# kuleshov-group/PlantCaduceus

Measured on AMD Instinct MI355X. Metric: 512-bp sequences/sec (zero-shot logits), PlantCaduceus_l32, higher is better.
Workload: dtype bf16; 1 GPU; PlantCaduceus_l32 (d_model=1024, n_layer=32) bf16 zero-shot SNP scoring: masked-LM forward of 1024 synthetic 512-bp windows per GPU per step (both strands), logits at index 255 -> softmax(a,c,g,t); synthetic checkpoint seed 1234; batch_per_gpu=1024, seq_len=512, parallelism=dp1 (batch-sharded, all_gather of [B,4])

## Files before the change

include/pcad.h:

```cpp
#ifndef PCAD_H
#define PCAD_H

#include <stddef.h>
#include <stdint.h>

#ifdef __cplusplus
extern "C" {
#endif

#define PCAD_VERSION 100
#define PCAD_MAX_VOCAB 8
#define PCAD_MAX_POSITIONS 16

typedef void* pcad_stream;
typedef struct pcad_engine* pcad_handle;

enum pcad_status {
    PCAD_OK = 0,
    PCAD_ERR_INVALID = -1,
    PCAD_ERR_UNBOUND = -2,
    PCAD_ERR_WORKSPACE = -3,
    PCAD_ERR_MISSING = -4,
    PCAD_ERR_HIP = -5
};
// ... 26 lines not shown
const char* pcad_last_error(void);
const char* pcad_build_hash(void);

int    pcad_create(const pcad_config* cfg, pcad_handle* out);
void   pcad_destroy(pcad_handle h);

int    pcad_set_option(pcad_handle h, const char* key, int64_t value);

enum pcad_status_bits { PCAD_STATUS_BAD_TOKEN = 1, PCAD_STATUS_BAD_POSITION = 2 };
int    pcad_set_status_buffer(pcad_handle h, int32_t* status);

size_t pcad_weight_arena_bytes(pcad_handle h);

int    pcad_bind_weights(pcad_handle h, const pcad_tensor* tensors, int n,
                         void* arena, size_t arena_bytes, pcad_stream stream);

size_t pcad_workspace_bytes(pcad_handle h, int batch, int seqlen);

int    pcad_forward(pcad_handle h, const int32_t* ids, int B, int L,
                    const int32_t* positions, int P,
                    void* hidden_out, float* logits_out,
                    void* workspace, size_t workspace_bytes, pcad_stream stream);

int    pcad_forward_at(pcad_handle h, const int32_t* ids, int B, int L, const int32_t* pos_per_seq,
                       void* hidden_out, float* logits_out,
                       void* workspace, size_t workspace_bytes, pcad_stream stream);

int    pcad_forward_all_hidden(pcad_handle h, const int32_t* ids, int B, int L,
                               void* all_hidden, void* hidden_out, float* logits_out,
                               void* workspace, size_t workspace_bytes, pcad_stream stream);

enum pcad_pooling { PCAD_POOL_MEAN = 0, PCAD_POOL_MAX = 1, PCAD_POOL_FIRST = 2, PCAD_POOL_LAST = 3 };
#define PCAD_MAX_LABELS 256
int    pcad_forward_pooled(pcad_handle h, const int32_t* ids, int B, int L, int pooling, const float* score_w, int num_labels,
                           float* pooled_out, float* logits_out, void* workspace, size_t workspace_bytes, pcad_stream stream);

enum pcad_kernel_class {
    PCAD_K_NORM = 0, PCAD_K_GEMM_IN, PCAD_K_CONV, PCAD_K_GEMM_X, PCAD_K_SCAN, PCAD_K_GEMM_OUT, PCAD_K_HEAD,
    PCAD_K_GEMM_OUT_RES,
    PCAD_K_RSTD,
    PCAD_NUM_KERNEL_CLASSES
};
typedef struct pcad_kernel_stat {
    char    name[32];
    int64_t launches;
    double  total_ms;
} pcad_kernel_stat;
int pcad_profile_enable(pcad_handle h, int on);
int pcad_profile_read(pcad_handle h, pcad_kernel_stat* out, int max_out);


int pcad_add_rmsnorm(const void* x, const void* residual_in, const float* weight,
                     void* y, void* residual_out, int64_t rows, int D, float eps,
                     int dtype, int res_dtype, pcad_stream stream);

int pcad_causal_conv1d_silu(const void* x, int64_t ldx, const float* w_fwd, const float* b_fwd,
                            const float* w_rev, const float* b_rev, void* y_fwd, void* y_rev,
                            int S, int L, int E, int dtype, pcad_stream stream);

size_t pcad_conv_xproj_scratch_bytes(int E, int dtype);
int pcad_conv_xproj_bidir(const void* x, const float* w_fwd, const float* b_fwd, const float* w_rev, const float* b_rev,
                          const void* Wx_fwd, const void* Wx_rev, void* scratch,
                          void* xc_fwd, void* dtl_fwd, float* bc_fwd, void* xc_rev, void* dtl_rev, float* bc_rev,
                          int S, int L, int E, int Rp, int dtype, pcad_stream stream);

int pcad_selective_scan(const void* u, const void* delta, const void* z, int64_t ldz, const float* bc,
                        const float* A, const float* Dskip, const float* delta_bias,
                        void* y, int S, int L, int E, int reverse, int accumulate,
                        int dtype, pcad_stream stream);

int pcad_selective_scan_dtproj(const void* u, const void* dt_low, int64_t lddt, const void* Wdt, int Rp,
                               const void* z, int64_t ldz, const float* bc,
                               const float* A, const float* Dskip, const float* delta_bias,
                               void* y, int S, int L, int E, int reverse, int accumulate,
                               int dtype, pcad_stream stream);

int pcad_gemm_nt(const void* A, int64_t lda, const void* W, int64_t ldw, void* C, int64_t ldc,
                 int64_t M, int N, int K, int dtype, int out_dtype, pcad_stream stream);

size_t pcad_gemm_nt_split_scratch_bytes(int64_t M, int N, int K);
int pcad_gemm_nt_split(const float* A, int64_t lda, const float* W, int64_t ldw, float* C, int64_t ldc, int64_t M, int N, int K,
                       void* scratch, size_t scratch_bytes, pcad_stream stream);

int pcad_gemm_nt_residual(const void* A, int64_t lda, const void* W, int64_t ldw, void* C, float* res, float* ssq,
                          int64_t M, int N, int K, int dtype, pcad_stream stream);

int pcad_gather_rows(const void* src, void* out, int B, int L, int E, const int32_t* positions, int P, int dtype,
                     pcad_stream stream);

int pcad_final_head(const void* h, const void* res, const float* norm_weight, const float* emb_f32, const int32_t* complement,
                    void* hidden_out, float* logits_out, int B, int L, int D, float eps, const int32_t* positions, int P,
                    const int32_t* pos_per_seq, int h_compact, const int32_t* ids, int32_t* status, int dtype, int res_dtype,
                    int res_fragment_layout, pcad_stream stream);

size_t pcad_pooled_head_scratch_bytes(int B, int L, int D, int pooling);
int pcad_pooled_head(const void* h, const void* res, const float* norm_weight, const float* score_w, int num_labels,
                     float* pooled_out, float* logits_out, int B, int L, int D, float eps, int pooling, const int32_t* ids,
                     int32_t* status, int dtype, int res_dtype, int res_fragment_layout, void* scratch, size_t scratch_bytes,
                     pcad_stream stream);

#ifdef __cplusplus
}
#endif
#endif
```

plantcaduceus_amd/csrc/api.hip:

```cpp
#include <hip/hip_runtime.h>

#include <cstdarg>
#include <cstdio>
#include <cstdlib>
#include <cstring>
#include <map>
#include <string>
#include <vector>

#include "../../include/pcad.h"
#include "build_hash.h"
#include "kernels.hpp"

using namespace pcad;

namespace {

thread_local char g_err[512] = "";

int fail(int code, const char* fmt, ...) {
    va_list ap;
    va_start(ap, fmt);
    vsnprintf(g_err, sizeof(g_err), fmt, ap);
    va_end(ap);
// ... 801 lines not shown
        return fail(PCAD_ERR_INVALID, "pcad_conv_xproj_bidir: null argument");
    if (dtype != PCAD_F32 && dtype != PCAD_BF16) return fail(PCAD_ERR_INVALID, "pcad_conv_xproj_bidir: bad dtype");
    if (Rp != 64 && Rp != 96) return fail(PCAD_ERR_INVALID, "pcad_conv_xproj_bidir: Rp must be 64 (dt_rank <= 64) or 96 (dt_rank 65..96)");
    const int64_t esz = dtype == PCAD_BF16 ? 2 : 4;
    if (S < 0 || L < 0 || E <= 0 || (E * esz) % 128)
        return fail(PCAD_ERR_INVALID, "pcad_conv_xproj_bidir: E * elem must be a multiple of 128 bytes");
    if (((int64_t)S * L + 16) * E * esz >= ((int64_t)1 << 32))
        return fail(PCAD_ERR_INVALID, "pcad_conv_xproj_bidir: (S*L + 16) * E * elem must be < 2^32 (32-bit in-tensor offsets)");
    if (S == 0 || L == 0) return PCAD_OK;
    hipStream_t s = (hipStream_t)stream;
    HIP_TRY(launch_pack_convw(w_fwd, b_fwd, w_rev, b_rev, (float*)scratch, E, dtype, s));
    HIP_TRY(launch_convx(x, (const float*)scratch, Wx_fwd, xc_fwd, dtl_fwd, bc_fwd, Wx_rev, xc_rev, dtl_rev, bc_rev, S, L, E,
                         dtype, s, Rp));
    return PCAD_OK;
}

static int scan_args_ok(const void* u, const float* bc, const float* A, const float* Dskip, const float* delta_bias,
                        void* y, int S, int L, int E) {
    if (!u || !bc || !A || !Dskip || !delta_bias || !y) return fail(PCAD_ERR_INVALID, "pcad_selective_scan: null argument");
    if (S < 0 || L < 0 || E <= 0 || E % 64) return fail(PCAD_ERR_INVALID, "pcad_selective_scan: E must be a multiple of 64");
    if (((uintptr_t)bc) % 16) return fail(PCAD_ERR_INVALID, "pcad_selective_scan: bc must be 16-byte aligned");
    return PCAD_OK;
}

int pcad_selective_scan(const void* u, const void* delta, const void* z, int64_t ldz, const float* bc, const float* A,
                        const float* Dskip, const float* delta_bias, void* y, int S, int L, int E, int reverse,
                        int accumulate, int dtype, pcad_stream stream) {
    if (!delta) return fail(PCAD_ERR_INVALID, "pcad_selective_scan: null delta");
    if (int rc = scan_args_ok(u, bc, A, Dskip, delta_bias, y, S, L, E)) return rc;
    if (S == 0 || L == 0) return PCAD_OK;
    HIP_TRY(launch_scan(u, z, ldz, delta, nullptr, 0, nullptr, 0, bc, A, 1.4426950408889634f, Dskip, delta_bias, y, S, L,
                        E, reverse != 0, accumulate, dtype, (hipStream_t)stream));
    return PCAD_OK;
}

int pcad_selective_scan_dtproj(const void* u, const void* dt_low, int64_t lddt, const void* Wdt, int Rp, const void* z,
                               int64_t ldz, const float* bc, const float* A, const float* Dskip,
                               const float* delta_bias, void* y, int S, int L, int E, int reverse, int accumulate,
                               int dtype, pcad_stream stream) {
    if (!dt_low || !Wdt) return fail(PCAD_ERR_INVALID, "pcad_selective_scan_dtproj: null dt_low / Wdt");
    if (Rp <= 0 || Rp % 32 || lddt < Rp || ((uintptr_t)dt_low) % 16 || ((uintptr_t)Wdt) % 16 ||
        (lddt * (dtype == PCAD_BF16 ? 2 : 4)) % 16)
        return fail(PCAD_ERR_INVALID, "pcad_selective_scan_dtproj: Rp must be a multiple of 32 (zero padded), rows 16-byte aligned");
    if (int rc = scan_args_ok(u, bc, A, Dskip, delta_bias, y, S, L, E)) return rc;
    if (S == 0 || L == 0) return PCAD_OK;
    HIP_TRY(launch_scan(u, z, ldz, nullptr, dt_low, lddt, Wdt, Rp, bc, A, 1.4426950408889634f, Dskip, delta_bias, y, S, L,
                        E, reverse != 0, accumulate, dtype, (hipStream_t)stream));
    return PCAD_OK;
}

int pcad_gemm_nt(const void* A, int64_t lda, const void* W, int64_t ldw, void* C, int64_t ldc, int64_t M, int N, int K,
                 int dtype, int out_dtype, pcad_stream stream) {
    if (!A || !W || !C) return fail(PCAD_ERR_INVALID, "pcad_gemm_nt: null argument");
    hipError_t err = launch_gemm_nt(A, lda, W, ldw, C, ldc, M, N, K, dtype, out_dtype, false, (hipStream_t)stream);
    if (err == hipErrorInvalidValue)
        return fail(PCAD_ERR_INVALID, "pcad_gemm_nt: K*elem must be a multiple of 128 bytes; A/W 16-byte aligned rows");
    if (err != hipSuccess) return fail(PCAD_ERR_HIP, "pcad_gemm_nt: %s", hipGetErrorString(err));
    return PCAD_OK;
}

size_t pcad_gemm_nt_split_scratch_bytes(int64_t M, int N, int K) {
    if (M <= 0 || N <= 0 || K <= 0) return 0;
    return align_up((size_t)M * 2 * K * 2) + align_up((size_t)N * 2 * K * 2);
}

int pcad_gemm_nt_split(const float* A, int64_t lda, const float* W, int64_t ldw, float* C, int64_t ldc, int64_t M, int N, int K,
                       void* scratch, size_t scratch_bytes, pcad_stream stream) {
    if (!A || !W || !C || !scratch) return fail(PCAD_ERR_INVALID, "pcad_gemm_nt_split: null argument");
    if (M < 0 || N <= 0 || K <= 0 || K % 64 || lda < K || ldw < K || ldc < N)
        return fail(PCAD_ERR_INVALID, "pcad_gemm_nt_split: K must be a multiple of 64; lda, ldw >= K; ldc >= N");
    if (((uintptr_t)scratch) % 256 || scratch_bytes < pcad_gemm_nt_split_scratch_bytes(M, N, K))
        return fail(PCAD_ERR_WORKSPACE, "pcad_gemm_nt_split: scratch must be 256-byte aligned and pcad_gemm_nt_split_scratch_bytes large");
    if (M == 0) return PCAD_OK;
    hipStream_t s = (hipStream_t)stream;
    void* As = scratch;
    void* Ws = (char*)scratch + align_up((size_t)M * 2 * K * 2);
    HIP_TRY(launch_split_rows(A, lda, As, M, K, false, false, s));
    HIP_TRY(launch_pack_split_w(W, PCAD_F32, ldw, Ws, N, K, s));
    hipError_t err = launch_gemm_nt(As, 2 * (int64_t)K, Ws, 2 * (int64_t)K, C, ldc, M, N, 3 * K, BF16, F32, false, s, false, K / 64);
    if (err != hipSuccess) return fail(PCAD_ERR_HIP, "pcad_gemm_nt_split: %s", hipGetErrorString(err));
    return PCAD_OK;
}

int pcad_gemm_nt_residual(const void* A, int64_t lda, const void* W, int64_t ldw, void* C, float* res, float* ssq, int64_t M, int N,
                          int K, int dtype, pcad_stream stream) {
    if (!A || !W || !res || !ssq || !C) return fail(PCAD_ERR_INVALID, "pcad_gemm_nt_residual: null argument");
    if (dtype != PCAD_F32 && dtype != PCAD_BF16) return fail(PCAD_ERR_INVALID, "pcad_gemm_nt_residual: bad dtype");
    if (M < 0 || N <= 0 || K <= 0 || M % 256 || N % 256 || M * (int64_t)N * 4 >= ((int64_t)1 << 32))
        return fail(PCAD_ERR_INVALID, "pcad_gemm_nt_residual: M and N must be multiples of 256 and M * N * 4 < 2^32");
    hipError_t err = launch_gemm_nt_res(A, lda, W, ldw, C, res, ssq, M, N, K, dtype, (hipStream_t)stream, false);
    if (err == hipErrorInvalidValue)
        return fail(PCAD_ERR_INVALID, "pcad_gemm_nt_residual: K*elem must be a multiple of 128 bytes; 16-byte aligned rows; tensors < 4 GiB");
    if (err != hipSuccess) return fail(PCAD_ERR_HIP, "pcad_gemm_nt_residual: %s", hipGetErrorString(err));
    return PCAD_OK;
}

static int positions_arg(const char* who, const int32_t* positions, int P, int L, Positions* pos) {
    if (P < 0 || P > PCAD_MAX_POSITIONS || (P > 0 && !positions)) return fail(PCAD_ERR_INVALID, "%s: bad positions (P=%d)", who, P);
    pos->n = P;
    for (int i = 0; i < 16; ++i) pos->p[i] = 0;
    for (int i = 0; i < P; ++i) {
        if (positions[i] < 0 || positions[i] >= L) return fail(PCAD_ERR_INVALID, "%s: position %d out of range [0,%d)", who, positions[i], L);
        pos->p[i] = positions[i];
    }
    return PCAD_OK;
}

int pcad_gather_rows(const void* src, void* out, int B, int L, int E, const int32_t* positions, int P, int dtype, pcad_stream stream) {
    if (!src || !out) return fail(PCAD_ERR_INVALID, "pcad_gather_rows: null argument");
    if (dtype != PCAD_F32 && dtype != PCAD_BF16) return fail(PCAD_ERR_INVALID, "pcad_gather_rows: bad dtype");
    if (B < 0 || L <= 0 || E <= 0 || (E * (dtype == PCAD_BF16 ? 2 : 4)) % 16 || P < 1)
        return fail(PCAD_ERR_INVALID, "pcad_gather_rows: bad shape (E * elem must be a multiple of 16 bytes, P >= 1)");
    Positions pos;
    if (int rc = positions_arg("pcad_gather_rows", positions, P, L, &pos)) return rc;
    if (B == 0) return PCAD_OK;
    HIP_TRY(launch_gather_rows(src, out, B, L, E, pos, dtype, false, (hipStream_t)stream));
    return PCAD_OK;
}

int pcad_final_head(const void* h, const void* res, const float* norm_weight, const float* emb_f32, const int32_t* complement,
                    void* hidden_out, float* logits_out, int B, int L, int D, float eps, const int32_t* positions, int P,
                    const int32_t* pos_per_seq, int h_compact, const int32_t* ids, int32_t* status, int dtype, int res_dtype,
                    int res_fragment_layout, pcad_stream stream) {
    if (!h || !res || !norm_weight || !emb_f32 || !complement) return fail(PCAD_ERR_INVALID, "pcad_final_head: null argument");
    if (res_fragment_layout && (res_dtype != PCAD_F32 || D % 256 || ((int64_t)2 * B * L) % 256))
        return fail(PCAD_ERR_INVALID, "pcad_final_head: the fragment layout needs an fp32 residual, D %% 256 == 0 and 2 B L %% 256 == 0");
    if ((dtype != PCAD_F32 && dtype != PCAD_BF16) || (res_dtype != PCAD_F32 && res_dtype != PCAD_BF16) || (dtype == PCAD_F32 && res_dtype != PCAD_F32))
        return fail(PCAD_ERR_INVALID, "pcad_final_head: bad dtype / res_dtype");
    if (B < 0 || L <= 0 || D <= 0 || D % 8 || D > 2048) return fail(PCAD_ERR_INVALID, "pcad_final_head: bad B / L / D");
    if (pos_per_seq && (positions || P)) return fail(PCAD_ERR_INVALID, "pcad_final_head: positions and pos_per_seq are exclusive");
    if (h_compact && (pos_per_seq || P == 0)) return fail(PCAD_ERR_INVALID, "pcad_final_head: h_compact needs a shared list of positions");
    Positions pos;
    if (int rc = positions_arg("pcad_final_head", positions, P, L, &pos)) return rc;
    if (B == 0) return PCAD_OK;
    HIP_TRY(launch_final_head(h, res, norm_weight, nullptr, emb_f32, complement, hidden_out, logits_out, B, L, D, eps, pos, pos_per_seq,
                              dtype, res_dtype, (hipStream_t)stream, h_compact != 0, ids, status, res_fragment_layout ? D : 0));
    return PCAD_OK;
}

size_t pcad_pooled_head_scratch_bytes(int B, int L, int D, int pooling) {
    if (B <= 0 || L <= 0 || D <= 0 || pooling < PCAD_POOL_MEAN || pooling > PCAD_POOL_LAST) return 0;
    return align_up(pool_partial_bytes(B, L, D, pooling));
}

int pcad_pooled_head(const void* h, const void* res, const float* norm_weight, const float* score_w, int num_labels,
                     float* pooled_out, float* logits_out, int B, int L, int D, float eps, int pooling, const int32_t* ids,
                     int32_t* status, int dtype, int res_dtype, int res_fragment_layout, void* scratch, size_t scratch_bytes,
                     pcad_stream stream) {
    if (!h || !res || !norm_weight || !scratch) return fail(PCAD_ERR_INVALID, "pcad_pooled_head: null argument");
    if (!pooled_out && !logits_out) return fail(PCAD_ERR_INVALID, "pcad_pooled_head: no output requested");
    if (logits_out && (!score_w || num_labels < 1 || num_labels > PCAD_MAX_LABELS))
        return fail(PCAD_ERR_INVALID, "pcad_pooled_head: logits need score_w and 1 <= num_labels <= %d", PCAD_MAX_LABELS);
    if (pooling < PCAD_POOL_MEAN || pooling > PCAD_POOL_LAST) return fail(PCAD_ERR_INVALID, "pcad_pooled_head: bad pooling %d", pooling);
    if (res_fragment_layout && (res_dtype != PCAD_F32 || D % 256 || ((int64_t)2 * B * L) % 256))
        return fail(PCAD_ERR_INVALID, "pcad_pooled_head: the fragment layout needs an fp32 residual, D %% 256 == 0 and 2 B L %% 256 == 0");
    if ((dtype != PCAD_F32 && dtype != PCAD_BF16) || (res_dtype != PCAD_F32 && res_dtype != PCAD_BF16) || (dtype == PCAD_F32 && res_dtype != PCAD_F32))
        return fail(PCAD_ERR_INVALID, "pcad_pooled_head: bad dtype / res_dtype");
    if (B < 0 || L <= 0 || D <= 0 || D % 8 || D > 2048) return fail(PCAD_ERR_INVALID, "pcad_pooled_head: bad B / L / D");
    if (B == 0) return PCAD_OK;
    if (((uintptr_t)scratch) % 256 || scratch_bytes < pcad_pooled_head_scratch_bytes(B, L, D, pooling))
        return fail(PCAD_ERR_WORKSPACE, "pcad_pooled_head: scratch must be 256-byte aligned and pcad_pooled_head_scratch_bytes large");
    HIP_TRY(launch_pooled_head(h, res, norm_weight, score_w, num_labels, pooled_out, logits_out, B, L, D, eps, pooling, ids, status,
                               dtype, res_dtype, res_fragment_layout ? D : 0, scratch, (hipStream_t)stream));
    return PCAD_OK;
}

// ... 2 lines not shown
```

plantcaduceus_amd/csrc/gemm.hip:

```cpp
#include <cstdlib>
#include <type_traits>

#include "common.hpp"
#include "kernels.hpp"

namespace pcad {

typedef __bf16 bf16x8_t __attribute__((ext_vector_type(8)));

constexpr int BM = 256, BN = 128, ROWB = 128;
constexpr int A_BYTES = BM * ROWB, W_BYTES = BN * ROWB;
constexpr int STAGE_BYTES = A_BYTES + W_BYTES;
constexpr int NSTAGE = 3;
constexpr int GEMM_LDS = NSTAGE * STAGE_BYTES;
constexpr int GEMM_THREADS = 512;
#ifndef PCAD_WALK_CONST
#define PCAD_WALK_CONST 8
#endif
constexpr int walk = PCAD_WALK_CONST;

__device__ __forceinline__ int ksplit_a(int kt, int nk) { return kt >= 2 * nk ? kt - 2 * nk : kt; }
__device__ __forceinline__ int ksplit_w(int kt, int nk) { return kt >= nk ? kt - nk : kt; }
__device__ __forceinline__ int key_a(int r) { return (r >> 1) & 7; }
__device__ __forceinline__ int key_w(int r) { return (((r >> 4) & 3) << 1) | ((r >> 1) & 1); }
// ... 801 lines not shown
                        *reinterpret_cast<u32x4*>(db + 64) = H;
                        __builtin_amdgcn_sched_barrier(0);
                        continue;
                    }
                }
                store8<OutT>(dst, lo);
                store8<OutT>(dst + 8, hi);
                __builtin_amdgcn_sched_barrier(0);
            }
        }
        if constexpr (EPI == EPI_RES) {
            const int np = N >> 7;
#pragma unroll
            for (int i = 0; i < 8; ++i) {
                float v = ss[i];
                v += __shfl_xor(v, 16, 64);
                v += __shfl_xor(v, 32, 64);
                if (lg == 0) epi.ssq[(mrow + i * 16) * np + (n0 >> 7) + wn] = v;
            }
        }
    };

    int tile = blockIdx.x;
    int64_t m0; int n0;
    tile_coords(tile, m0, n0);
    set_pa(m0);
    set_pw(n0);
    load_rscale(m0);
    a_issue(0); a_advance();
    w_issue(0); w_advance();
    a_issue(1); a_advance();
    w_issue(1); w_advance();
    asm volatile("s_waitcnt vmcnt(16)" ::: "memory");
    __builtin_amdgcn_s_barrier();
    asm volatile("" ::: "memory");
    u32x4 fa0[8], fw0[8], fa1[8], fw1[8];
    load_frags(0, 0, 0, fa0, fw0);
    int sa = 0, sw = 0, kt = 0;
    auto mainloop = [&](auto slot) __attribute__((always_inline)) {
    while (true) {
        const int sa_n = sa == 2 ? 0 : sa + 1;
        const int sa_f = sa == 0 ? 2 : sa - 1;
        if constexpr (EPI == EPI_RES) {
            if (kt == 0) {
                const float* tb = res_tile_base(m0, n0);
#pragma unroll
                for (int i = 0; i < 8; ++i) { load_res_group(tb, i, 0); load_res_group(tb, i, 1); }
                kstep(fa0, fw0, fa1, fw1, sa, sw, 1, true, sa_f, std::integral_constant<int, 2>{}, slot);
            } else {
                kstep(fa0, fw0, fa1, fw1, sa, sw, 1, true, sa_f, std::integral_constant<int, 0>{}, slot);
            }
        } else {
            if (kt == 0) kstep(fa0, fw0, fa1, fw1, sa, sw, 1, true, sa_f, std::integral_constant<int, 1>{}, slot);
            else kstep(fa0, fw0, fa1, fw1, sa, sw, 1, true, sa_f, std::integral_constant<int, 0>{}, slot);
        }
        a_advance();
        asm volatile("s_waitcnt vmcnt(8) lgkmcnt(0)" ::: "memory");
        __builtin_amdgcn_s_barrier();
        asm volatile("" ::: "memory");
        kstep(fa1, fw1, fa0, fw0, sa_n, sw ^ 1, 0, false, sw, std::integral_constant<int, 0>{}, slot);
        w_advance();
        sa = sa_n;
        sw ^= 1;
        if (kt + 1 < nkt) {
            ++kt;
        } else {
            epilogue(m0, n0);
            tile += gstride;
            if (tile >= nblk) break;
            tile_coords(tile, m0, n0);
            load_rscale(m0);
            kt = 0;
        }
    }
    };
#ifdef PCAD_GEMM_STAGGER
    if (wave == 0) mainloop(std::integral_constant<int, 0>{});
    else if (wave == 1) mainloop(std::integral_constant<int, 1>{});
    else if (wave == 2) mainloop(std::integral_constant<int, 2>{});
    else mainloop(std::integral_constant<int, 3>{});
#else
    mainloop(std::integral_constant<int, kDmaSlot>{});
#endif
    asm volatile("s_waitcnt vmcnt(0)" ::: "memory");
}

static int persistent_grid(int nblk) {
    const int cap = device_cu_count() / 8 * 8;
    return nblk < cap ? nblk : cap;
}

template <typename T, typename OutT, bool ROUND>
static hipError_t launch_gemm_t(const void* A, int64_t lda, const void* W, int64_t ldw, void* C, int64_t ldc,
                                int64_t M, int N, int K, hipStream_t s, bool a_blocked, int ksplit = 0) {
    const int tiles_m = (int)((M + BM - 1) / BM), tiles_n = (N + BN - 1) / BN;
    const bool vec = ((ldc * (int64_t)sizeof(OutT)) % 16 == 0) && (((uintptr_t)C) % 16 == 0);
    dim3 grid((unsigned)persistent_grid(tiles_m * tiles_n)), block(GEMM_THREADS);
    if (vec) {
        auto kfn = gemm_nt_kernel<T, OutT, ROUND, true, false>;
        if (hipError_t ae = ensure_dynamic_lds((const void*)kfn, GEMM_LDS)) return ae;
        hipLaunchKernelGGL(kfn, grid, block, GEMM_LDS, s, (const T*)A, lda, (const T*)W, ldw, (OutT*)C, ldc, M, N, K,
                           tiles_m, tiles_n, (float*)nullptr, (int64_t)0, 0, (int)a_blocked, ksplit);
    } else {
        auto kfn = gemm_nt_kernel<T, OutT, ROUND, false, false>;
        if (hipError_t ae = ensure_dynamic_lds((const void*)kfn, GEMM_LDS)) return ae;
        hipLaunchKernelGGL(kfn, grid, block, GEMM_LDS, s, (const T*)A, lda, (const T*)W, ldw, (OutT*)C, ldc, M, N, K,
                           tiles_m, tiles_n, (float*)nullptr, (int64_t)0, 0, (int)a_blocked, ksplit);
    }
    return hipGetLastError();
}

template <typename T>
static hipError_t launch_gemm_split_t(const void* A, int64_t lda, const void* W, int64_t ldw, void* C, int64_t ldc,
                                      float* C2, int64_t ldc2, int nsplit, int64_t M, int N, int K, hipStream_t s,
                                      bool a_blocked) {
    const int tiles_m = (int)((M + BM - 1) / BM), tiles_n = (N + BN - 1) / BN;
    dim3 grid((unsigned)persistent_grid(tiles_m * tiles_n)), block(GEMM_THREADS);
    auto kfn = gemm_nt_kernel<T, T, false, true, true>;
    if (hipError_t ae = ensure_dynamic_lds((const void*)kfn, GEMM_LDS)) return ae;
    hipLaunchKernelGGL(kfn, grid, block, GEMM_LDS, s, (const T*)A, lda, (const T*)W, ldw, (T*)C, ldc, M, N, K, tiles_m,
                       tiles_n, C2, ldc2, nsplit, (int)a_blocked, 0);
    return hipGetLastError();
}

hipError_t launch_gemm_nt_split(const void* A, int64_t lda, const void* W, int64_t ldw, void* C, int64_t ldc, float* C2,
                                int64_t ldc2, int nsplit, int64_t M, int N, int K, int dt, hipStream_t s, bool a_blocked) {
    if (M <= 0 || N <= 0) return hipSuccess;
    const int esz = dt == BF16 ? 2 : 4;
    if (K <= 0 || (K * esz) % ROWB || nsplit % 16 || (N - nsplit) % 16) return hipErrorInvalidValue;
    if ((lda * esz) % 16 || (ldw * esz) % 16 || ((uintptr_t)A) % 16 || ((uintptr_t)W) % 16) return hipErrorInvalidValue;
    if ((ldc * esz) % 16 || ((uintptr_t)C) % 16 || (ldc2 * 4) % 16 || ((uintptr_t)C2) % 16) return hipErrorInvalidValue;
    if (a_blocked && (lda * esz) % 128) return hipErrorInvalidValue;
    if (dt == BF16) return launch_gemm_split_t<bf16_t>(A, lda, W, ldw, C, ldc, C2, ldc2, nsplit, M, N, K, s, a_blocked);
    return launch_gemm_split_t<float>(A, lda, W, ldw, C, ldc, C2, ldc2, nsplit, M, N, K, s, a_blocked);
}

template <typename T>
static bool quad_ok(int64_t lda, int64_t ldw, int64_t M, int N, bool two, int nsplit) {
    const int64_t esz_ = (int64_t)sizeof(T);
    return M % BM2 == 0 && N % BN2 == 0 && (!two || nsplit % 64 == 0) && M * lda * esz_ < ((int64_t)1 << 32) - 65536 &&
           (int64_t)N * ldw * esz_ < ((int64_t)1 << 32) - 65536;
}

template <typename T, typename OutT = T>
static hipError_t launch_gemm256_t(const void* A, int64_t lda, const void* W, int64_t ldw, void* C, int64_t ldc, int64_t M,
                                   int N, int K, hipStream_t s, bool a_blocked, void* C2 = nullptr, int nsplit = 0,
                                   bool out_blocked = false, int epi_kind = EPI_NONE, GemmEpi epi = GemmEpi{nullptr, nullptr, nullptr},
                                   int ksplit = 0) {
    const int tiles_m = (int)((M + BM2 - 1) / BM2), tiles_n = (N + BN2 - 1) / BN2;
    dim3 grid((unsigned)persistent_grid(tiles_m * tiles_n)), block(GEMM_THREADS);
    static const bool quad = dev_env("PCAD_GEMM_NOQUAD") == nullptr;
    static const bool epi_swap = dev_env("PCAD_GEMM_EPI_PLAIN") == nullptr;
    const bool qok = quad_ok<T>(lda, ldw, M, N, C2 != nullptr, nsplit);
    if (epi_kind != EPI_NONE && !qok) return hipErrorInvalidValue;
#define PCAD_LAUNCH_Q(EPIK)                                                                                                     \
    do {                                                                                                                        \
        auto kq = gemm256q_kernel<T, OutT, EPIK>;                                                                               \
        if (hipError_t ae = ensure_dynamic_lds((const void*)kq, GEMM3_LDS)) return ae;                                          \
        hipLaunchKernelGGL(kq, grid, dim3(GEMMQ_THREADS), GEMM3_LDS, s, (const T*)A, lda, (const T*)W, ldw, (OutT*)C, ldc, M, N, K, \
                           tiles_m, tiles_n, (int)a_blocked, (OutT*)C2, nsplit, (int)out_blocked, (int)epi_swap, epi, ksplit); \
                                                                                             \
        return hipGetLastError();                                                                                               \
    } while (0)
    if constexpr (std::is_same<T, OutT>::value) {
        if (epi_kind == EPI_SCALE) PCAD_LAUNCH_Q(EPI_SCALE);
        if (epi_kind == EPI_RES) PCAD_LAUNCH_Q(EPI_RES);
    } else if (epi_kind != EPI_NONE) {
        return hipErrorInvalidValue;
    }
    if (quad && qok) PCAD_LAUNCH_Q(EPI_NONE);
#undef PCAD_LAUNCH_Q
    auto kr = gemm256r_kernel<T, OutT>;
    if (hipError_t ae = ensure_dynamic_lds((const void*)kr, GEMM3_LDS)) return ae;
    hipLaunchKernelGGL(kr, grid, block, GEMM3_LDS, s, (const T*)A, lda, (const T*)W, ldw, (OutT*)C, ldc, M, N, K, tiles_m,
                       tiles_n, (int)a_blocked, (OutT*)C2, nsplit, (int)out_blocked, ksplit);
    return hipGetLastError();
}

hipError_t launch_gemm_nt_two(const void* A, int64_t lda, const void* W, int64_t ldw, void* C1, void* C2, int nsplit,
                              bool out_blocked, int64_t M, int N, int K, int dt, hipStream_t s, const float* rscale, int out_dt, int ksplit) {
    if (M <= 0 || N <= 0) return hipSuccess;
    const int esz = dt == BF16 ? 2 : 4;
    if (out_dt < 0) out_dt = dt;
    const int osz = out_dt == BF16 ? 2 : 4;
    if (K <= 0 || (K * esz) % ROWB || nsplit % 16 || N % 16 || nsplit <= 0 || nsplit >= N) return hipErrorInvalidValue;
    if ((lda * esz) % 16 || (ldw * esz) % 16 || ((uintptr_t)A) % 16 || ((uintptr_t)W) % 16) return hipErrorInvalidValue;
    if (((uintptr_t)C1) % 16 || ((uintptr_t)C2) % 16) return hipErrorInvalidValue;
    if (out_blocked && ((nsplit * osz) % 128 || ((N - nsplit) * osz) % 128)) return hipErrorInvalidValue;
    const int ek = rscale ? EPI_SCALE : EPI_NONE;
    const GemmEpi epi{rscale, nullptr, nullptr};
    if (out_dt != dt) {
        if (dt != BF16 || out_dt != F32 || rscale) return hipErrorInvalidValue;
        if (ksplit && (ksplit < 0 || K != 3 * ksplit * (ROWB / 2))) return hipErrorInvalidValue;
        return launch_gemm256_t<bf16_t, float>(A, lda, W, ldw, C1, nsplit, M, N, K, s, false, C2, nsplit, out_blocked, EPI_NONE, epi, ksplit);
    }
    if (ksplit) return hipErrorInvalidValue;
    if (dt == BF16) return launch_gemm256_t<bf16_t>(A, lda, W, ldw, C1, nsplit, M, N, K, s, false, C2, nsplit, out_blocked, ek, epi);
    return launch_gemm256_t<float>(A, lda, W, ldw, C1, nsplit, M, N, K, s, false, C2, nsplit, out_blocked, ek, epi);
}

bool gemm_fold_shapes_ok(int64_t M, int D, int E, int dt) {
    const int64_t esz = dt == BF16 ? 2 : 4;
    const int Dp = fold_padded_width(D);
    const bool in_ok = dt == BF16 ? quad_ok<bf16_t>(Dp, D, M, 2 * E, true, E) : quad_ok<float>(Dp, D, M, 2 * E, true, E);
    const bool out_ok = dt == BF16 ? quad_ok<bf16_t>(E, E, M, Dp, false, 0) : quad_ok<float>(E, E, M, Dp, false, 0);
    return in_ok && out_ok && (D * esz) % ROWB == 0 && (E * esz) % ROWB == 0 && M * (int64_t)Dp * 4 < ((int64_t)1 << 32);
}

hipError_t launch_gemm_nt_res(const void* A, int64_t lda, const void* W, int64_t ldw, void* C, float* res, float* ssq, int64_t M,
                              int N, int K, int dt, hipStream_t s, bool a_blocked) {
    if (M <= 0 || N <= 0) return hipSuccess;
    const int esz = dt == BF16 ? 2 : 4;
    if (K <= 0 || (K * esz) % ROWB || !res || !ssq || !C) return hipErrorInvalidValue;
    if ((lda * esz) % 16 || (ldw * esz) % 16 || ((uintptr_t)A) % 16 || ((uintptr_t)W) % 16 || ((uintptr_t)res) % 16) return hipErrorInvalidValue;
    if (a_blocked && (lda * esz) % 128) return hipErrorInvalidValue;
    const GemmEpi epi{nullptr, res, ssq};
    if (dt == BF16) return launch_gemm256_t<bf16_t>(A, lda, W, ldw, C, N, M, N, K, s, a_blocked, nullptr, 0, false, EPI_RES, epi);
    return launch_gemm256_t<float>(A, lda, W, ldw, C, N, M, N, K, s, a_blocked, nullptr, 0, false, EPI_RES, epi);
}

hipError_t launch_gemm_nt(const void* A, int64_t lda, const void* W, int64_t ldw, void* C, int64_t ldc, int64_t M,
                          int N, int K, int dt, int out_dt, bool round_bf16, hipStream_t s, bool a_blocked, int ksplit) {
    if (M <= 0 || N <= 0) return hipSuccess;
    const int esz = dt == BF16 ? 2 : 4;
    if (K <= 0 || (K * esz) % ROWB) return hipErrorInvalidValue;
    if (ksplit && (ksplit < 0 || dt != BF16 || out_dt != F32 || round_bf16 || K != 3 * ksplit * (ROWB / 2))) return hipErrorInvalidValue;
    if ((lda * esz) % 16 || (ldw * esz) % 16 || ((uintptr_t)A) % 16 || ((uintptr_t)W) % 16)
        return hipErrorInvalidValue;
    if (a_blocked && (lda * esz) % 128) return hipErrorInvalidValue;
    static const bool no256 = dev_env("PCAD_GEMM_NO256") != nullptr;
    const int osz = out_dt == BF16 ? 2 : 4;
    const bool big = !no256 && M >= 2048 && N >= 512 && N % 16 == 0 && (out_dt == dt || (dt == BF16 && out_dt == F32 && !round_bf16)) &&
                     (ldc * osz) % 16 == 0 && ((uintptr_t)C) % 16 == 0;
    if (big) {
        if (dt == BF16 && out_dt == F32)
            return launch_gemm256_t<bf16_t, float>(A, lda, W, ldw, C, ldc, M, N, K, s, a_blocked, nullptr, 0, false, EPI_NONE, GemmEpi{nullptr, nullptr, nullptr}, ksplit);
        if (dt == BF16) return launch_gemm256_t<bf16_t>(A, lda, W, ldw, C, ldc, M, N, K, s, a_blocked);
        return launch_gemm256_t<float>(A, lda, W, ldw, C, ldc, M, N, K, s, a_blocked);
    }
    if (dt == BF16 && out_dt == BF16)
        return launch_gemm_t<bf16_t, bf16_t, false>(A, lda, W, ldw, C, ldc, M, N, K, s, a_blocked);
    if (dt == BF16 && out_dt == F32)
        return round_bf16 ? launch_gemm_t<bf16_t, float, true>(A, lda, W, ldw, C, ldc, M, N, K, s, a_blocked)
                          : launch_gemm_t<bf16_t, float, false>(A, lda, W, ldw, C, ldc, M, N, K, s, a_blocked, ksplit);
    if (dt == F32 && out_dt == F32)
        return launch_gemm_t<float, float, false>(A, lda, W, ldw, C, ldc, M, N, K, s, a_blocked);
    return hipErrorInvalidValue;
}

}
```

plantcaduceus_amd/engine.py:

```python
from __future__ import annotations

import ctypes as C
import os
import subprocess
from typing import Dict, Optional, Sequence

import torch

_HERE = os.path.dirname(os.path.abspath(__file__))
LIB_PATH = os.environ.get("PCAD_LIB") or os.path.join(_HERE, "libpcad.so")
CSRC = os.path.join(_HERE, "csrc")

PCAD_F32, PCAD_BF16 = 0, 1
_DT = {torch.float32: PCAD_F32, torch.bfloat16: PCAD_BF16}


class PcadConfig(C.Structure):
    _fields_ = [
        ("d_model", C.c_int32), ("n_layer", C.c_int32), ("d_state", C.c_int32), ("d_conv", C.c_int32),
        ("expand", C.c_int32), ("dt_rank", C.c_int32), ("vocab", C.c_int32), ("eps", C.c_float),
        ("dtype", C.c_int32), ("residual_in_fp32", C.c_int32), ("complement", C.c_int32 * 8),
    ]


class PcadKernelStat(C.Structure):
    _fields_ = [("name", C.c_char * 32), ("launches", C.c_int64), ("total_ms", C.c_double)]


class PcadTensor(C.Structure):
    _fields_ = [("name", C.c_char_p), ("data", C.c_void_p), ("dtype", C.c_int32), ("ndim", C.c_int32),
                ("shape", C.c_int64 * 4)]


SIGNATURES = {
    "pcad_version": (C.c_int, []),
    "pcad_last_error": (C.c_char_p, []),
    "pcad_build_hash": (C.c_char_p, []),
    "pcad_set_status_buffer": (C.c_int, [C.c_void_p, C.c_void_p]),
    "pcad_create": (C.c_int, [C.POINTER(PcadConfig), C.POINTER(C.c_void_p)]),
    "pcad_destroy": (None, [C.c_void_p]),
    "pcad_set_option": (C.c_int, [C.c_void_p, C.c_char_p, C.c_int64]),
    "pcad_weight_arena_bytes": (C.c_size_t, [C.c_void_p]),
    "pcad_bind_weights": (C.c_int, [C.c_void_p, C.POINTER(PcadTensor), C.c_int, C.c_void_p, C.c_size_t, C.c_void_p]),
    "pcad_workspace_bytes": (C.c_size_t, [C.c_void_p, C.c_int, C.c_int]),
    "pcad_forward": (C.c_int, [C.c_void_p, C.c_void_p, C.c_int, C.c_int, C.POINTER(C.c_int32), C.c_int,
                               C.c_void_p, C.c_void_p, C.c_void_p, C.c_size_t, C.c_void_p]),
    "pcad_forward_at": (C.c_int, [C.c_void_p, C.c_void_p, C.c_int, C.c_int, C.c_void_p, C.c_void_p, C.c_void_p,
                                  C.c_void_p, C.c_size_t, C.c_void_p]),
    "pcad_forward_all_hidden": (C.c_int, [C.c_void_p, C.c_void_p, C.c_int, C.c_int, C.c_void_p, C.c_void_p,
                                          C.c_void_p, C.c_void_p, C.c_size_t, C.c_void_p]),
    "pcad_profile_enable": (C.c_int, [C.c_void_p, C.c_int]),
    "pcad_profile_read": (C.c_int, [C.c_void_p, C.POINTER(PcadKernelStat), C.c_int]),
    "pcad_add_rmsnorm": (C.c_int, [C.c_void_p, C.c_void_p, C.c_void_p, C.c_void_p, C.c_void_p, C.c_int64, C.c_int,
                                   C.c_float, C.c_int, C.c_int, C.c_void_p]),
    "pcad_causal_conv1d_silu": (C.c_int, [C.c_void_p, C.c_int64, C.c_void_p, C.c_void_p, C.c_void_p, C.c_void_p,
                                          C.c_void_p, C.c_void_p, C.c_int, C.c_int, C.c_int, C.c_int, C.c_void_p]),
    "pcad_conv_xproj_scratch_bytes": (C.c_size_t, [C.c_int, C.c_int]),
    "pcad_conv_xproj_bidir": (C.c_int, [C.c_void_p] * 14 + [C.c_int, C.c_int, C.c_int, C.c_int, C.c_int, C.c_void_p]),
    "pcad_selective_scan": (C.c_int, [C.c_void_p, C.c_void_p, C.c_void_p, C.c_int64, C.c_void_p, C.c_void_p,
                                      C.c_void_p, C.c_void_p, C.c_void_p, C.c_int, C.c_int, C.c_int, C.c_int,
                                      C.c_int, C.c_int, C.c_void_p]),
    "pcad_selective_scan_dtproj": (C.c_int, [C.c_void_p, C.c_void_p, C.c_int64, C.c_void_p, C.c_int, C.c_void_p,
                                             C.c_int64, C.c_void_p, C.c_void_p, C.c_void_p, C.c_void_p, C.c_void_p,
                                             C.c_int, C.c_int, C.c_int, C.c_int, C.c_int, C.c_int, C.c_void_p]),
    "pcad_gemm_nt": (C.c_int, [C.c_void_p, C.c_int64, C.c_void_p, C.c_int64, C.c_void_p, C.c_int64, C.c_int64,
                               C.c_int, C.c_int, C.c_int, C.c_int, C.c_void_p]),
    "pcad_gemm_nt_residual": (C.c_int, [C.c_void_p, C.c_int64, C.c_void_p, C.c_int64, C.c_void_p, C.c_void_p, C.c_void_p,
                                        C.c_int64, C.c_int, C.c_int, C.c_int, C.c_void_p]),
    "pcad_gemm_nt_split_scratch_bytes": (C.c_size_t, [C.c_int64, C.c_int, C.c_int]),
    "pcad_gemm_nt_split": (C.c_int, [C.c_void_p, C.c_int64, C.c_void_p, C.c_int64, C.c_void_p, C.c_int64, C.c_int64, C.c_int, C.c_int,
                                     C.c_void_p, C.c_size_t, C.c_void_p]),
    "pcad_gather_rows": (C.c_int, [C.c_void_p, C.c_void_p, C.c_int, C.c_int, C.c_int, C.POINTER(C.c_int32), C.c_int, C.c_int,
                                   C.c_void_p]),
    "pcad_final_head": (C.c_int, [C.c_void_p, C.c_void_p, C.c_void_p, C.c_void_p, C.c_void_p, C.c_void_p, C.c_void_p,
                                  C.c_int, C.c_int, C.c_int, C.c_float, C.POINTER(C.c_int32), C.c_int, C.c_void_p, C.c_int,
                                  C.c_void_p, C.c_void_p, C.c_int, C.c_int, C.c_int, C.c_void_p]),
    "pcad_forward_pooled": (C.c_int, [C.c_void_p, C.c_void_p, C.c_int, C.c_int, C.c_int, C.c_void_p, C.c_int, C.c_void_p,
                                      C.c_void_p, C.c_void_p, C.c_size_t, C.c_void_p]),
    "pcad_pooled_head_scratch_bytes": (C.c_size_t, [C.c_int, C.c_int, C.c_int, C.c_int]),
    "pcad_pooled_head": (C.c_int, [C.c_void_p, C.c_void_p, C.c_void_p, C.c_void_p, C.c_int, C.c_void_p, C.c_void_p, C.c_int,
                                   C.c_int, C.c_int, C.c_float, C.c_int, C.c_void_p, C.c_void_p, C.c_int, C.c_int, C.c_int,
                                   C.c_void_p, C.c_size_t, C.c_void_p]),
}

POOLING = {"mean": 0, "max": 1, "first": 2, "last": 3}
MAX_LABELS = 256

_lib = None

STATUS_BAD_TOKEN, STATUS_BAD_POSITION = 1, 2


def source_hash() -> str:
    import importlib.util
    spec = importlib.util.spec_from_file_location("_pcad_source_hash", os.path.join(CSRC, "source_hash.py"))
    mod = importlib.util.module_from_spec(spec)
    spec.loader.exec_module(mod)
    return mod.source_hash(CSRC)


def build_library(force: bool = False) -> str:
    if force:
        subprocess.run(["make", "-C", CSRC, "clean"], check=True, capture_output=True)
    r = subprocess.run(["make", "-C", CSRC, "-j", "6"], capture_output=True, text=True)
    if r.returncode != 0:
        raise RuntimeError("building libpcad.so failed:\n" + r.stdout[-4000:] + "\n" + r.stderr[-4000:])
    return LIB_PATH


def load_library():
    global _lib
    if _lib is not None:
        return _lib
    if not os.path.exists(LIB_PATH):
        raise RuntimeError(
            f"{LIB_PATH} not found: the MI355X HIP extension is not built. Run "
            "`python -c 'import __graft_entry__ as g; g.build()'` (or `make -C plantcaduceus_amd/csrc`). "
            "There is deliberately no CPU fallback.")
    lib = C.CDLL(LIB_PATH)
    for name, (res, args) in SIGNATURES.items():
        fn = getattr(lib, name)
        fn.restype = res
        fn.argtypes = args
    if os.path.exists(os.path.join(CSRC, "source_hash.py")) and os.environ.get("PCAD_ALLOW_STALE") != "1":
        built, have = lib.pcad_build_hash().decode(), source_hash()
        if built != have:
            raise RuntimeError(
                f"{LIB_PATH} was built from other kernel sources (pcad_build_hash {built}, sources {have}): rebuild it with "
                "`make -C plantcaduceus_amd/csrc` / `__graft_entry__.build()` (PCAD_ALLOW_STALE=1 overrides, for A/B of old builds)")
    _lib = lib
    return lib


def _check(code: int, what: str):
    if code != 0:
        msg = load_library().pcad_last_error()
        raise RuntimeError(f"{what} failed ({code}): {msg.decode() if msg else ''}")


def _stream_ptr() -> int:
    return torch.cuda.current_stream().cuda_stream


def _require_gpu(t: torch.Tensor, name: str):
    if not t.is_cuda:
        raise RuntimeError(f"{name} must live on a ROCm device (got {t.device}); the MI355X engine has no CPU path")


class Engine:
# ... 197 lines not shown
```

Measured before the change: 1210 sequences/s.

## Add persistent ping-pong 256x256 bf16 GEMM for split in-projection

```diff
diff --git a/include/pcad.h b/include/pcad.h
--- a/include/pcad.h
+++ b/include/pcad.h
@@ -132,6 +132,9 @@
 int pcad_gemm_nt_split(const float* A, int64_t lda, const float* W, int64_t ldw, float* C, int64_t ldc, int64_t M, int N, int K,
                        void* scratch, size_t scratch_bytes, pcad_stream stream);
 
+int pcad_gemm_nt_two(const void* A, int64_t lda, const void* W, int64_t ldw, void* X, void* Z, int nsplit, int blocked,
+                     int64_t M, int N, int K, const float* rscale, int dtype, pcad_stream stream);
+
 int pcad_gemm_nt_residual(const void* A, int64_t lda, const void* W, int64_t ldw, void* C, float* res, float* ssq,
                           int64_t M, int N, int K, int dtype, pcad_stream stream);
 
diff --git a/plantcaduceus_amd/csrc/api.hip b/plantcaduceus_amd/csrc/api.hip
--- a/plantcaduceus_amd/csrc/api.hip
+++ b/plantcaduceus_amd/csrc/api.hip
@@ -907,6 +907,19 @@
     return PCAD_OK;
 }
 
+int pcad_gemm_nt_two(const void* A, int64_t lda, const void* W, int64_t ldw, void* X, void* Z, int nsplit, int blocked,
+                     int64_t M, int N, int K, const float* rscale, int dtype, pcad_stream stream) {
+    if (!A || !W || !X || !Z) return fail(PCAD_ERR_INVALID, "pcad_gemm_nt_two: null argument");
+    if (dtype != PCAD_F32 && dtype != PCAD_BF16) return fail(PCAD_ERR_INVALID, "pcad_gemm_nt_two: bad dtype");
+    if (M < 0 || N <= 0 || K <= 0 || M % 256 || N % 256 || nsplit <= 0 || nsplit >= N || nsplit % 64)
+        return fail(PCAD_ERR_INVALID, "pcad_gemm_nt_two: M, N multiples of 256, 0 < nsplit < N a multiple of 64");
+    hipError_t err = launch_gemm_nt_two(A, lda, W, ldw, X, Z, nsplit, blocked != 0, M, N, K, dtype, (hipStream_t)stream, rscale, -1, 0);
+    if (err == hipErrorInvalidValue)
+        return fail(PCAD_ERR_INVALID, "pcad_gemm_nt_two: K*elem must be a multiple of 128 bytes; 16-byte aligned rows; A, W < 4 GiB");
+    if (err != hipSuccess) return fail(PCAD_ERR_HIP, "pcad_gemm_nt_two: %s", hipGetErrorString(err));
+    return PCAD_OK;
+}
+
 int pcad_gemm_nt_residual(const void* A, int64_t lda, const void* W, int64_t ldw, void* C, float* res, float* ssq, int64_t M, int N,
                           int K, int dtype, pcad_stream stream) {
     if (!A || !W || !res || !ssq || !C) return fail(PCAD_ERR_INVALID, "pcad_gemm_nt_residual: null argument");
diff --git a/plantcaduceus_amd/csrc/gemm.hip b/plantcaduceus_amd/csrc/gemm.hip
--- a/plantcaduceus_amd/csrc/gemm.hip
+++ b/plantcaduceus_amd/csrc/gemm.hip
@@ -907,6 +907,264 @@
 #else
     mainloop(std::integral_constant<int, kDmaSlot>{});
 #endif
+    asm volatile("s_waitcnt vmcnt(0)" ::: "memory");
+}
+
+__device__ __forceinline__ f32x4 acc_read(const f32x4& c) {
+    f32x4 v;
+#pragma unroll
+    for (int e = 0; e < 4; ++e) {
+        float x;
+        asm volatile("v_accvgpr_read_b32 %0, %1" : "=v"(x) : "a"(c[e]));
+        v[e] = x;
+    }
+    return v;
+}
+constexpr int kPingPongWaitDma = 6;
+
+template <int EPI>
+__global__ __launch_bounds__(GEMM_THREADS, 2) void gemm256p_kernel(const bf16_t* __restrict__ A, int64_t lda,
+                                                                   const bf16_t* __restrict__ W, int64_t ldw,
+                                                                   bf16_t* __restrict__ C1, bf16_t* __restrict__ C2, int nsplit,
+                                                                   int64_t M, int N, int K, int tiles_m, int tiles_n,
+                                                                   int out_blocked, int epi_swap, GemmEpi epi) {
+    extern __shared__ __attribute__((aligned(16))) char smem[];
+    const int tid = threadIdx.x;
+    const int lane = tid & 63;
+    const int wave = __builtin_amdgcn_readfirstlane(tid >> 6);
+    const int gstride = (int)gridDim.x;
+    const int nblk = tiles_m * tiles_n;
+    const int nkt = (K * (int)sizeof(bf16_t)) / ROWB;
+    if ((int)blockIdx.x >= nblk) return;
+    const int my_tiles = (nblk - (int)blockIdx.x + gstride - 1) / gstride;
+    const int G = my_tiles * nkt;
+
+    auto tile_coords = [&](int tile, int64_t& m0, int& n0) __attribute__((always_inline)) {
+        const int xcd = tile & 7, idx = tile >> 3;
+        const int q = nblk >> 3, r = nblk & 7;
+        const int logical = (xcd < r ? xcd * (q + 1) : r * (q + 1) + (xcd - r) * q) + idx;
+        if (walk & 256) {
+            const int tm = logical / tiles_n;
+            m0 = (int64_t)tm * BM2;
+            n0 = (logical - tm * tiles_n) * BN2;
+            return;
+        }
+        const int group_m = walk & 255;
+        const int gsz = group_m * tiles_n;
+        const int g = logical / gsz;
+        const int first_m = g * group_m;
+        const int gm = min(group_m, tiles_m - first_m);
+        const int in_g = logical - g * gsz;
+        m0 = (int64_t)(first_m + in_g % gm) * BM2;
+        n0 = (in_g / gm) * BN2;
+    };
+
+    uint32_t a_lo[4], w_lo[4];
+#pragma unroll
+    for (int p = 0; p < 4; ++p) {
+        const int row = wave * 32 + p * 8 + (lane >> 3);
+        a_lo[p] = (uint32_t)((int64_t)row * lda * 2 + (((lane & 7) ^ key_a(row)) << 4));
+        w_lo[p] = (uint32_t)((int64_t)row * ldw * 2 + (((lane & 7) ^ key_w(row)) << 4));
+    }
+    uint32_t a_base, w_base;
+    auto set_pa = [&](int64_t m0) __attribute__((always_inline)) { a_base = (uint32_t)(m0 * lda * 2); };
+    auto set_pw = [&](int n0) __attribute__((always_inline)) { w_base = (uint32_t)((int64_t)n0 * ldw * 2); };
+    int a_tile = blockIdx.x, a_kt = 0, a_g = 0;
+    int w_tile = blockIdx.x, w_kt = 0, w_g = 0;
+    auto a_piece = [&](int sa, int p) __attribute__((always_inline)) {
+        blds16(A, a_lo[p], a_base + (uint32_t)a_kt * (uint32_t)ROWB, smem + sa * A2_BYTES + (wave * 32 + p * 8) * ROWB);
+    };
+    auto w_piece = [&](int sw, int p) __attribute__((always_inline)) {
+        blds16(W, w_lo[p], w_base + (uint32_t)w_kt * (uint32_t)ROWB, smem + GEMM3_OFF_W + sw * W2_BYTES + (wave * 32 + p * 8) * ROWB);
+    };
+    auto a_advance = [&]() __attribute__((always_inline)) {
+        if (a_g + 1 < G) {
+            ++a_g;
+            if (++a_kt == nkt) {
+                a_kt = 0;
+                a_tile += gstride;
+                int64_t m0; int n0;
+                tile_coords(a_tile, m0, n0);
+                set_pa(m0);
+            }
+        }
+    };
+    auto w_advance = [&]() __attribute__((always_inline)) {
+        if (w_g + 1 < G) {
+            ++w_g;
+            if (++w_kt == nkt) {
+                w_kt = 0;
+                w_tile += gstride;
+                int64_t m0; int n0;
+                tile_coords(w_tile, m0, n0);
+                set_pw(n0);
+            }
+        }
+    };
+
+    const int wm = wave >> 2, wn = wave & 3;
+    const int li = lane & 15, lg = lane >> 4;
+    const int ra = wm * 128 + li;
+    const int rw = wn * 64 + (li >> 2) * 16 + (li & 3);
+    const int a_fo = ra * ROWB + ((lg ^ key_a(ra)) << 4);
+    const int w_fo = GEMM3_OFF_W + rw * ROWB + ((lg ^ key_w(rw)) << 4);
+    u32x4 fa[8], fwl[4], fwh[4];
+    auto read_a = [&](int sa, int half) __attribute__((always_inline)) {
+#pragma unroll
+        for (int kk = 0; kk < 2; ++kk) {
+            const char* b = smem + ((sa * A2_BYTES + a_fo) ^ (kk << 6)) + half * 4 * 2048;
+#pragma unroll
+            for (int i = 0; i < 4; ++i) fa[kk * 4 + i] = *reinterpret_cast<const u32x4*>(b + i * 2048);
+        }
+    };
+    auto read_w = [&](int sw, int half, u32x4 (&fw)[4]) __attribute__((always_inline)) {
+#pragma unroll
+        for (int kk = 0; kk < 2; ++kk) {
+            const char* b = smem + ((sw * W2_BYTES + w_fo) ^ (kk << 6)) + half * 2 * 512;
+#pragma unroll
+            for (int j = 0; j < 2; ++j) fw[kk * 2 + j] = *reinterpret_cast<const u32x4*>(b + j * 512);
+        }
+    };
+
+    f32x4 acc[8][4];
+    auto phase_mma = [&](int mh, int nh, const u32x4 (&fw)[4], auto first_tag) __attribute__((always_inline)) {
+        constexpr bool FIRST = decltype(first_tag)::value;
+        asm volatile("" ::: "memory");
+        __builtin_amdgcn_sched_barrier(0);
+        __builtin_amdgcn_s_barrier();
+        asm volatile("s_waitcnt lgkmcnt(0)" ::: "memory");
+        __builtin_amdgcn_sched_barrier(0);
+        __builtin_amdgcn_s_setprio(1);
+#pragma unroll
+        for (int kk = 0; kk < 2; ++kk)
+#pragma unroll
+            for (int i = 0; i < 4; ++i)
+#pragma unroll
+                for (int j = 0; j < 2; ++j) {
+                    if (FIRST && kk == 0) MmaAcc<bf16_t>::run0(fw[kk * 2 + j], fa[kk * 4 + i], acc[mh * 4 + i][nh * 2 + j]);
+                    else MmaAcc<bf16_t>::run(fw[kk * 2 + j], fa[kk * 4 + i], acc[mh * 4 + i][nh * 2 + j]);
+                }
+        __builtin_amdgcn_s_setprio(0);
+        __builtin_amdgcn_s_barrier();
+        asm volatile("" ::: "memory");
+        __builtin_amdgcn_sched_barrier(0);
+    };
+    int sa = 0;
+    auto ktile = [&](auto sw_tag, auto first_tag) __attribute__((always_inline)) {
+        constexpr int SW = (int)decltype(sw_tag)::value;
+        const int sa2 = sa == 0 ? 2 : sa - 1;
+        read_a(sa, 0);
+        read_w(SW, 0, fwl);
+        w_piece(SW ^ 1, 2); w_piece(SW ^ 1, 3);
+        w_advance();
+        phase_mma(0, 0, fwl, first_tag);
+        read_w(SW, 1, fwh);
+        a_piece(sa2, 0); a_piece(sa2, 1);
+        phase_mma(0, 1, fwh, first_tag);
+        read_a(sa, 1);
+        a_piece(sa2, 2); a_piece(sa2, 3);
+        a_advance();
+        phase_mma(1, 1, fwh, first_tag);
+        w_piece(SW, 0); w_piece(SW, 1);
+        asm volatile("s_waitcnt vmcnt(%0)" ::"n"(kPingPongWaitDma) : "memory");
+        phase_mma(1, 0, fwl, first_tag);
+        sa = sa == 2 ? 0 : sa + 1;
+    };
+
+    const int swap_fix = (((lg & 1) * 16 + (lg >> 1) * 8) - lg * 16) * 2;
+    float rs[8];
+    auto load_rscale = [&](int64_t m0) __attribute__((always_inline)) {
+        if constexpr (EPI == EPI_SCALE) {
+            const float* sb = epi.rscale + (m0 + wm * 128);
+            const uint32_t vo = (uint32_t)li * 4u;
+            gload_v32<0>(rs[0], vo, sb);   gload_v32<64>(rs[1], vo, sb);  gload_v32<128>(rs[2], vo, sb); gload_v32<192>(rs[3], vo, sb);
+            gload_v32<256>(rs[4], vo, sb); gload_v32<320>(rs[5], vo, sb); gload_v32<384>(rs[6], vo, sb); gload_v32<448>(rs[7], vo, sb);
+        }
+    };
+    auto epilogue = [&](int64_t m0, int n0) __attribute__((always_inline)) {
+        const int64_t mrow = m0 + wm * 128 + li;
+        if constexpr (EPI == EPI_SCALE) wait_vmcnt_regs<kPingPongWaitDma>(rs);
+        const int nbase = n0 + wn * 64;
+        const bool second = nbase >= nsplit;
+        const int width = second ? N - nsplit : nsplit;
+        const int col = (second ? nbase - nsplit : nbase) + lg * 16;
+        char* base = reinterpret_cast<char*>(second ? C2 : C1);
+        char* lane_dst;
+        int64_t row_step;
+        if (out_blocked) {
+            lane_dst = base + blocked_off(mrow, (int64_t)col * 2, ((int64_t)width * 2) >> 7);
+            row_step = 2 * ((((int64_t)width * 2) >> 7) << 10);
+        } else {
+            lane_dst = base + (mrow * width + col) * 2;
+            row_step = 16 * (int64_t)width * 2;
+        }
+#pragma unroll
+        for (int i = 0; i < 8; ++i) {
+            f32x4 t0 = acc_read(acc[i][0]), t1 = acc_read(acc[i][1]), t2 = acc_read(acc[i][2]), t3 = acc_read(acc[i][3]);
+            if constexpr (EPI == EPI_SCALE) { t0 *= rs[i]; t1 *= rs[i]; t2 *= rs[i]; t3 *= rs[i]; }
+            float lo[8], hi[8];
+#pragma unroll
+            for (int rr = 0; rr < 4; ++rr) {
+                lo[rr] = t0[rr]; lo[4 + rr] = t1[rr];
+                hi[rr] = t2[rr]; hi[4 + rr] = t3[rr];
+            }
+            bf16_t* dst = reinterpret_cast<bf16_t*>(lane_dst + i * row_step);
+            if (epi_swap) {
+                u32x4 L, H;
+#pragma unroll
+                for (int d = 0; d < 4; ++d) {
+                    const auto sw = __builtin_amdgcn_permlane32_swap(pack_bf16x2(lo[2 * d], lo[2 * d + 1]), pack_bf16x2(hi[2 * d], hi[2 * d + 1]), false, false);
+                    L[d] = sw[0]; H[d] = sw[1];
+                }
+                char* db = reinterpret_cast<char*>(dst) + swap_fix;
+                *reinterpret_cast<u32x4*>(db) = L;
+                *reinterpret_cast<u32x4*>(db + 64) = H;
+            } else {
+                store8<bf16_t>(dst, lo);
+                store8<bf16_t>(dst + 8, hi);
+            }
+            __builtin_amdgcn_sched_barrier(0);
+        }
+    };
+
+    int tile = blockIdx.x;
+    int64_t m0; int n0;
+    tile_coords(tile, m0, n0);
+    set_pa(m0);
+    set_pw(n0);
+    load_rscale(m0);
+#pragma unroll
+    for (int p = 0; p < 4; ++p) a_piece(0, p);
+    a_advance();
+#pragma unroll
+    for (int p = 0; p < 4; ++p) w_piece(0, p);
+    w_advance();
+#pragma unroll
+    for (int p = 0; p < 4; ++p) a_piece(1, p);
+    a_advance();
+    w_piece(1, 0); w_piece(1, 1);
+    asm volatile("s_waitcnt vmcnt(%0)" ::"n"(kPingPongWaitDma) : "memory");
+    __builtin_amdgcn_s_barrier();
+    if (wm == 1) __builtin_amdgcn_s_barrier();
+    asm volatile("" ::: "memory");
+    using F = std::integral_constant<bool, false>;
+    using T1 = std::integral_constant<bool, true>;
+    using S0 = std::integral_constant<int, 0>;
+    using S1 = std::integral_constant<int, 1>;
+    while (true) {
+        ktile(S0{}, T1{});
+        ktile(S1{}, F{});
+        for (int kt = 2; kt < nkt; kt += 2) {
+            ktile(S0{}, F{});
+            ktile(S1{}, F{});
+        }
+        epilogue(m0, n0);
+        tile += gstride;
+        if (tile >= nblk) break;
+        tile_coords(tile, m0, n0);
+        load_rscale(m0);
+    }
+    if (wm == 0) __builtin_amdgcn_s_barrier();
     asm volatile("s_waitcnt vmcnt(0)" ::: "memory");
 }
 
@@ -1020,6 +1278,17 @@
         return launch_gemm256_t<bf16_t, float>(A, lda, W, ldw, C1, nsplit, M, N, K, s, false, C2, nsplit, out_blocked, EPI_NONE, epi, ksplit);
     }
     if (ksplit) return hipErrorInvalidValue;
+    static const bool inproj_q = dev_env("PCAD_GEMM_INPROJ_Q") != nullptr;
+    if (dt == BF16 && !inproj_q && quad_ok<bf16_t>(lda, ldw, M, N, true, nsplit) && (K * esz / ROWB) % 2 == 0) {
+        static const bool epi_swap = dev_env("PCAD_GEMM_EPI_PLAIN") == nullptr;
+        const int tiles_m = (int)(M / BM2), tiles_n = N / BN2;
+        dim3 grid((unsigned)persistent_grid(tiles_m * tiles_n)), block(GEMM_THREADS);
+        auto kp = rscale ? gemm256p_kernel<EPI_SCALE> : gemm256p_kernel<EPI_NONE>;
+        if (hipError_t ae = ensure_dynamic_lds((const void*)kp, GEMM3_LDS)) return ae;
+        hipLaunchKernelGGL(kp, grid, block, GEMM3_LDS, s, (const bf16_t*)A, lda, (const bf16_t*)W, ldw, (bf16_t*)C1, (bf16_t*)C2, nsplit,
+                           M, N, K, tiles_m, tiles_n, (int)out_blocked, (int)epi_swap, epi);
+        return hipGetLastError();
+    }
     if (dt == BF16) return launch_gemm256_t<bf16_t>(A, lda, W, ldw, C1, nsplit, M, N, K, s, false, C2, nsplit, out_blocked, ek, epi);
     return launch_gemm256_t<float>(A, lda, W, ldw, C1, nsplit, M, N, K, s, false, C2, nsplit, out_blocked, ek, epi);
 }
diff --git a/plantcaduceus_amd/engine.py b/plantcaduceus_amd/engine.py
--- a/plantcaduceus_amd/engine.py
+++ b/plantcaduceus_amd/engine.py
@@ -65,6 +65,8 @@
                                              C.c_int, C.c_int, C.c_int, C.c_int, C.c_int, C.c_int, C.c_void_p]),
     "pcad_gemm_nt": (C.c_int, [C.c_void_p, C.c_int64, C.c_void_p, C.c_int64, C.c_void_p, C.c_int64, C.c_int64,
                                C.c_int, C.c_int, C.c_int, C.c_int, C.c_void_p]),
+    "pcad_gemm_nt_two": (C.c_int, [C.c_void_p, C.c_int64, C.c_void_p, C.c_int64, C.c_void_p, C.c_void_p, C.c_int, C.c_int,
+                                   C.c_int64, C.c_int, C.c_int, C.c_void_p, C.c_int, C.c_void_p]),
     "pcad_gemm_nt_residual": (C.c_int, [C.c_void_p, C.c_int64, C.c_void_p, C.c_int64, C.c_void_p, C.c_void_p, C.c_void_p,
                                         C.c_int64, C.c_int, C.c_int, C.c_int, C.c_void_p]),
     "pcad_gemm_nt_split_scratch_bytes": (C.c_size_t, [C.c_int64, C.c_int, C.c_int]),
```

After: 1216 sequences/s, median of 6. No clear change (+0.6%).
